# burchim/EfficientConformer

Hardware: AMD Instinct MI355X
Metric: audio-frames/sec through encoder, EffConformerCTC-Small, 1/2/4/8 GPU (higher is better)
Workload: dtype bf16; 1 GPU; EfficientConformerCTCSmall: bf16 operands / fp32 accumulate, B=256 utterances/GPU (the largest single-GPU batch measured; SURVEY.md 8d lists B in {4, 32, 128}: --batch 128 is 0.79 x this rate, profiles/r5_31_bench_b128.json), lognormal 1.5-16 s (LibriSpeech-shaped), sorted desc; ragged: every utterance at its own length in one concatenated row space per row range (no pad frames; outputs = the refe; global_batch=256, streams_per_gpu=3, parallelism=dp1 (utterance shards), row_ranges=3 ragged row range(s) per GPU, cut for equal valid frames

## Files before the change

### efficientconformer_amd/csrc/mel.hip

```cpp
#include "kernels.h"

#ifdef MEL_PK_BUILD
#define launch_mel launch_mel_pk_unused
#define launch_mel_debug launch_mel_debug_pk
#define MEL_NS mel_pk_build
#else
#define MEL_NS
#endif

namespace MEL_NS {

constexpr int NFFT = 512;
constexpr int FRAMES_PER_BLOCK = 32;
constexpr int MAX_MELS = 128;
constexpr int P1 = 72;
constexpr int P2 = 68;
constexpr int MAX_FBW = 768;

__device__ __forceinline__ float2 cmul(float2 a, float2 b) { return make_float2(a.x * b.x - a.y * b.y, a.x * b.y + a.y * b.x); }
__device__ __forceinline__ float2 cadd(float2 a, float2 b) { return make_float2(a.x + b.x, a.y + b.y); }
__device__ __forceinline__ float2 csub(float2 a, float2 b) { return make_float2(a.x - b.x, a.y - b.y); }
__device__ __forceinline__ float2 mul_mi(float2 a) { return make_float2(a.y, -a.x); }
__device__ __forceinline__ float2 mul_pi(float2 a) { return make_float2(-a.y, a.x); }

__device__ __forceinline__ void dft8(float2 (&v)[8]) {
    const float r = 0.70710678118654752f;
    float2 a[4], b[4];
#pragma unroll
    for (int j = 0; j < 4; ++j) { a[j] = cadd(v[j], v[j + 4]); b[j] = csub(v[j], v[j + 4]); }
    b[1] = make_float2(r * (b[1].x + b[1].y), r * (b[1].y - b[1].x));
    b[2] = mul_mi(b[2]);
    b[3] = make_float2(r * (b[3].y - b[3].x), -r * (b[3].x + b[3].y));
    {
        const float2 s0 = cadd(a[0], a[2]), s1 = cadd(a[1], a[3]), d0 = csub(a[0], a[2]), d1 = csub(a[1], a[3]);
        v[0] = cadd(s0, s1); v[4] = csub(s0, s1); v[2] = cadd(d0, mul_mi(d1)); v[6] = cadd(d0, mul_pi(d1));
    }
    {
        const float2 s0 = cadd(b[0], b[2]), s1 = cadd(b[1], b[3]), d0 = csub(b[0], b[2]), d1 = csub(b[1], b[3]);
        v[1] = cadd(s0, s1); v[5] = csub(s0, s1); v[3] = cadd(d0, mul_mi(d1)); v[7] = cadd(d0, mul_pi(d1));
    }
}

__device__ __forceinline__ float2 reread(const float2* p) {
    const volatile float* q = reinterpret_cast<const volatile float*>(p);
    return make_float2(q[0], q[1]);
}

template <int V, int MM>
__global__ __launch_bounds__(256) void mel_kernel(const float* __restrict__ audio, int L, MelTables tb, int hop,
                                                  int n_mels, int Tm, int normalize, float mean, float inv_std,
                                                  float* __restrict__ mel, unsigned int* __restrict__ dbg,
                                                  const int64_t* __restrict__ rag_len = nullptr) {
    constexpr int CAN = (V & 1) ? 512 : 0;
    constexpr int WBUF = 8 * P1 * 8;
    constexpr int O_SBUF = CAN * 4, O_POST = O_SBUF + 4 * WBUF, O_STW = O_POST + CAN * 4, O_SWIN = O_STW + (NFFT / 2) * 8,
                  O_SOUT = O_SWIN + NFFT * 4, O_SFW = O_SOUT + MM * (FRAMES_PER_BLOCK + 1) * 4, O_END = O_SFW + MAX_FBW * 4;
    static_assert(8 * P1 >= NFFT && P1 >= P2 && 8 * P1 * 2 >= 264 + NFFT / 2 + 1, "one buffer holds Z[512], the step-2 layout and the two power spectra");
    __shared__ __attribute__((aligned(16))) char lds[O_END];
    float2* stw = reinterpret_cast<float2*>(lds + O_STW);
    float* swin = reinterpret_cast<float*>(lds + O_SWIN);
    float (*sout)[FRAMES_PER_BLOCK + 1] = reinterpret_cast<float (*)[FRAMES_PER_BLOCK + 1]>(lds + O_SOUT);
    float* sfw = reinterpret_cast<float*>(lds + O_SFW);
    if constexpr ((V & 1) != 0) {
        unsigned int* c0 = reinterpret_cast<unsigned int*>(lds), *c1 = reinterpret_cast<unsigned int*>(lds + O_POST);
        for (int i = threadIdx.x; i < CAN; i += 256) { c0[i] = 0xC0FFEE00u + i; c1[i] = 0xBADC0DE0u + i; }
    }
    auto hand_off = [&]() __attribute__((always_inline)) { if constexpr ((V & 4) != 0) __syncthreads(); else wave_sync(); };
    unsigned int bad[8] = {0, 0, 0, 0, 0, 0, 0, 0};
    auto neq = [](float2 a, float2 b) { return (__float_as_uint(a.x) != __float_as_uint(b.x)) | (__float_as_uint(a.y) != __float_as_uint(b.y)); };
    const int tiles = (Tm + FRAMES_PER_BLOCK - 1) / FRAMES_PER_BLOCK;
    const int b = blockIdx.x / tiles, t0 = (blockIdx.x % tiles) * FRAMES_PER_BLOCK;
    const int Lb = rag_len ? (int)rag_len[b] : L;
    const int Tmb = rag_len ? Lb / hop + 1 : Tm;
    if (t0 >= Tmb) return;
    const int tid = threadIdx.x, lane = tid & 63, wave = tid >> 6;
    const bool fw_lds = tb.fb_nnz <= MAX_FBW;
    {
        static_assert(NFFT == 512 && MAX_FBW == 768, "two / three passes of 256 threads");
        const float2 w = tb.twiddle[tid];
        const float wn0 = tb.window[tid], wn1 = tb.window[tid + 256];
        float f[3];
#pragma unroll
        for (int j = 0; j < 3; ++j) { const int i = tid + 256 * j; f[j] = tb.fb_weight[i < tb.fb_nnz ? i : (tb.fb_nnz > 0 ? tb.fb_nnz - 1 : 0)]; }
        stw[tid] = w;
        swin[tid] = wn0; swin[tid + 256] = wn1;
        if (fw_lds) {
#pragma unroll
            for (int j = 0; j < 3; ++j) if (tid + 256 * j < tb.fb_nnz) sfw[tid + 256 * j] = f[j];
        }
    }
    int fs0[2], fcnt[2], foff[2];
#pragma unroll
    for (int j = 0; j < 2; ++j) {
        const int m = (threadIdx.x & 63) + 64 * j, mc = m < n_mels ? m : n_mels - 1;
        fs0[j] = tb.fb_start[mc]; fcnt[j] = m < n_mels ? tb.fb_count[mc] : 0; foff[j] = tb.fb_offset[mc];
    }
    __syncthreads();
    float2* A = reinterpret_cast<float2*>(lds + O_SBUF + wave * WBUF);
    float2* B = A;
    auto tw = [&](int m) __attribute__((always_inline)) {
        float2 w = stw[m & 255];
        const uint32_t sg = (uint32_t)(m & 256) << 23;
        w.x = __uint_as_float(__float_as_uint(w.x) ^ sg); w.y = __uint_as_float(__float_as_uint(w.y) ^ sg);
        return w;
    };
    const float* a = audio + (size_t)b * L;

    auto gather = [&](int ta, float (&xa)[8], float (&xb)[8]) __attribute__((always_inline)) {
#pragma unroll
        for (int j = 0; j < 8; ++j) {
            const int n = lane + 64 * j;
            int sa = ta * hop - NFFT / 2 + n, sb = sa + hop;
            sa = sa < 0 ? -sa : sa; sa = sa >= Lb ? 2 * (Lb - 1) - sa : sa; sa = sa < 0 ? 0 : (sa >= Lb ? Lb - 1 : sa);
            sb = sb < 0 ? -sb : sb; sb = sb >= Lb ? 2 * (Lb - 1) - sb : sb; sb = sb < 0 ? 0 : (sb >= Lb ? Lb - 1 : sb);
            xa[j] = a[sa]; xb[j] = a[sb];
        }
    };
    float nxa[8], nxb[8];
    gather(t0 + wave * (FRAMES_PER_BLOCK / 4), nxa, nxb);
    for (int it = 0; it < FRAMES_PER_BLOCK / 8; ++it) {
        const int fl = wave * (FRAMES_PER_BLOCK / 4) + 2 * it;
        const int ta = t0 + fl, tbb = ta + 1;
        float2 v[8];
#pragma unroll
        for (int j = 0; j < 8; ++j) {
            const float w = swin[lane + 64 * j];
            v[j] = make_float2(ta < Tmb ? nxa[j] * w : 0.f, tbb < Tmb ? nxb[j] * w : 0.f);
        }
        bool nza = false, nzb = false;
#pragma unroll
        for (int j = 0; j < 8; ++j) { nza |= v[j].x != 0.f; nzb |= v[j].y != 0.f; }
        const bool live_a = __builtin_amdgcn_ballot_w64(nza) != 0, live_b = __builtin_amdgcn_ballot_w64(nzb) != 0;
        if (it + 1 < FRAMES_PER_BLOCK / 8) gather(ta + 2, nxa, nxb);
        {
            const int n2 = lane >> 3;
            dft8(v);
#pragma unroll
            for (int k1 = 0; k1 < 8; ++k1) { v[k1] = cmul(v[k1], tw((8 * n2 * k1) & 511)); A[k1 * P1 + lane] = v[k1]; }
        }
        hand_off();
        if constexpr ((V & 2) != 0) {
#pragma unroll
            for (int k1 = 0; k1 < 8; ++k1) bad[1] += neq(A[k1 * P1 + lane], v[k1]);
        }
        {
            const int k1 = lane >> 3, n3 = lane & 7;
#pragma unroll
            for (int n2 = 0; n2 < 8; ++n2) v[n2] = A[k1 * P1 + n2 * 8 + n3];
            if constexpr ((V & 2) != 0) {
                __builtin_amdgcn_fence(__ATOMIC_ACQUIRE, "wavefront");
#pragma unroll
                for (int n2 = 0; n2 < 8; ++n2) bad[2] += neq(reread(&A[k1 * P1 + n2 * 8 + n3]), v[n2]);
            }
            dft8(v);
#pragma unroll
            for (int k2 = 0; k2 < 8; ++k2) { v[k2] = cmul(v[k2], tw((n3 * (k1 + 8 * k2)) & 511)); B[n3 * P2 + k1 + 8 * k2] = v[k2]; }
        }
        hand_off();
        if constexpr ((V & 2) != 0) {
            const int k1 = lane >> 3, n3 = lane & 7;
#pragma unroll
            for (int k2 = 0; k2 < 8; ++k2) bad[3] += neq(B[n3 * P2 + k1 + 8 * k2], v[k2]);
        }
#pragma unroll
        for (int n3 = 0; n3 < 8; ++n3) v[n3] = B[n3 * P2 + lane];
        if constexpr ((V & 2) != 0) {
            __builtin_amdgcn_fence(__ATOMIC_ACQUIRE, "wavefront");
#pragma unroll
            for (int n3 = 0; n3 < 8; ++n3) bad[4] += neq(reread(&B[n3 * P2 + lane]), v[n3]);
        }
        dft8(v);
#pragma unroll
        for (int k3 = 0; k3 < 8; ++k3) A[lane + 64 * k3] = v[k3];
        hand_off();
        if constexpr ((V & 2) != 0) {
#pragma unroll
            for (int k3 = 0; k3 < 8; ++k3) bad[5] += neq(A[lane + 64 * k3], v[k3]);
        }
        float* Pa = reinterpret_cast<float*>(B);
        float* Pb = Pa + 264;
        float2 zz[5], zcc[5];
#pragma unroll
        for (int j = 0; j < 5; ++j) {
            const int k = lane + 64 * j, kc = k <= NFFT / 2 ? k : NFFT / 2;
            zz[j] = A[kc]; zcc[j] = A[(NFFT - kc) & (NFFT - 1)];
            if constexpr ((V & 2) != 0) {
                __builtin_amdgcn_fence(__ATOMIC_ACQUIRE, "wavefront");
                bad[6] += neq(reread(&A[kc]), zz[j]) + neq(reread(&A[(NFFT - kc) & (NFFT - 1)]), zcc[j]);
            }
        }
        hand_off();
#pragma unroll
        for (int j = 0; j < 5; ++j) {
            const int k = lane + 64 * j;
            if (k <= NFFT / 2) {
                const float2 z = zz[j], zc = zcc[j];
                const float ar = 0.5f * (z.x + zc.x), ai = 0.5f * (z.y - zc.y);
                const float br = 0.5f * (z.y + zc.y), bi = 0.5f * (zc.x - z.x);
                Pa[k] = live_a ? ar * ar + ai * ai : 0.f;
                Pb[k] = live_b ? br * br + bi * bi : 0.f;
            }
        }
        hand_off();
#pragma unroll
        for (int mj = 0; mj < 2; ++mj) {
            const int m = lane + 64 * mj;
            if (m >= n_mels) break;
            const int s0 = fs0[mj], cnt = fcnt[mj], off = foff[mj];
            float ya = 0.f, yb = 0.f;
            if (fw_lds) {
                for (int j0 = 0; j0 < cnt; j0 += 4) {
                    float wj[4], pa[4], pb[4];
#pragma unroll
                    for (int e = 0; e < 4; ++e) {
                        const int j = j0 + e, jc = j < cnt ? j : cnt - 1;
                        wj[e] = j < cnt ? sfw[off + jc] : 0.f;
                        pa[e] = Pa[s0 + jc]; pb[e] = Pb[s0 + jc];
                    }
#pragma unroll
                    for (int e = 0; e < 4; ++e) { ya = fmaf(pa[e], wj[e], ya); yb = fmaf(pb[e], wj[e], yb); }
                }
            } else {
                const float* w = tb.fb_weight + off;
                for (int j = 0; j < cnt; ++j) { const float wj = w[j]; ya = fmaf(Pa[s0 + j], wj, ya); yb = fmaf(Pb[s0 + j], wj, yb); }
            }
            ya = logf(ya + 1e-9f); yb = logf(yb + 1e-9f);
            if (normalize) { ya = (ya - mean) * inv_std; yb = (yb - mean) * inv_std; }
            sout[m][fl] = ya;
            sout[m][fl + 1] = yb;
        }
        hand_off();
    }
    __syncthreads();
    for (int i = tid; i < n_mels * FRAMES_PER_BLOCK; i += 256) {
        const int m = i / FRAMES_PER_BLOCK, fl = i - m * FRAMES_PER_BLOCK;
        if (t0 + fl < Tmb) mel[((size_t)b * n_mels + m) * Tm + t0 + fl] = sout[m][fl];
    }
    if constexpr ((V & 1) != 0) {
        const unsigned int* c0 = reinterpret_cast<const unsigned int*>(lds), *c1 = reinterpret_cast<const unsigned int*>(lds + O_POST);
        for (int i = threadIdx.x; i < CAN; i += 256) bad[0] += (c0[i] != 0xC0FFEE00u + i) + (c1[i] != 0xBADC0DE0u + i);
    }
    if constexpr (V != 0) {
#pragma unroll
        for (int i = 0; i < 8; ++i) if (bad[i]) atomicAdd(dbg + i, bad[i]);
    }
}

}
#ifdef MEL_PK_BUILD
using namespace mel_pk_build;
#endif

int launch_mel(const float* audio, int B, int L, const MelTables& t, int n_fft, int hop, int n_mels, int Tm,
               int normalize, float mean, float std, float* mel, hipStream_t s, const int64_t* ragged_len) {
    if (B <= 0) return 0;
    if (n_fft != NFFT || n_mels > MAX_MELS || L <= n_fft / 2) return -2;
    const int tiles = (Tm + FRAMES_PER_BLOCK - 1) / FRAMES_PER_BLOCK;
    if (n_mels <= 80)
        hipLaunchKernelGGL((mel_kernel<0, 80>), dim3(B * tiles), dim3(256), 0, s, audio, L, t, hop, n_mels, Tm, normalize, mean,
                           1.0f / std, mel, (unsigned int*)nullptr, ragged_len);
    else
        hipLaunchKernelGGL((mel_kernel<0, MAX_MELS>), dim3(B * tiles), dim3(256), 0, s, audio, L, t, hop, n_mels, Tm, normalize, mean,
                           1.0f / std, mel, (unsigned int*)nullptr, ragged_len);
    return hipGetLastError() == hipSuccess ? 0 : -1;
}

#if defined(EFFCONF_DEBUG_ABI) || defined(MEL_PK_BUILD)
int launch_mel_debug(int variant, int extra_lds, const float* audio, int B, int L, const MelTables& t, int n_fft, int hop, int n_mels,
                     int Tm, int normalize, float mean, float std, float* mel, unsigned int* dbg, hipStream_t s) {
    if (B <= 0) return 0;
    if (n_fft != NFFT || n_mels > MAX_MELS || L <= n_fft / 2) return -2;
#ifndef MEL_PK_BUILD
    if (variant & 8) return launch_mel_debug_pk(variant & 7, extra_lds, audio, B, L, t, n_fft, hop, n_mels, Tm, normalize, mean, std, mel, dbg, s);
#endif
    const int tiles = (Tm + FRAMES_PER_BLOCK - 1) / FRAMES_PER_BLOCK;
#define MEL_DBG_CASE(VV) case VV: { static LdsAttr attr; ensure_dynamic_lds(reinterpret_cast<const void*>(&mel_kernel<VV, MAX_MELS>), extra_lds, attr); \
        hipLaunchKernelGGL((mel_kernel<VV, MAX_MELS>), dim3(B * tiles), dim3(256), extra_lds, s, audio, L, t, hop, n_mels, Tm, normalize, mean, 1.0f / std, mel, dbg, (const int64_t*)nullptr); break; }
    switch (variant) {
        MEL_DBG_CASE(0) MEL_DBG_CASE(1) MEL_DBG_CASE(2) MEL_DBG_CASE(3) MEL_DBG_CASE(4) MEL_DBG_CASE(5) MEL_DBG_CASE(6) MEL_DBG_CASE(7)
        default: return -2;
    }
#undef MEL_DBG_CASE
    return hipGetLastError() == hipSuccess ? 0 : -1;
}
#endif
```

Before: 61.85 million mel-frames/s (valid, 10 ms hop).

## Streamline mel kernel: fast-path audio gather, overlap table loads, simplify filterbank loop

Adds a fast path for interior frames that loads audio contiguously without reflect-padding index math, and falls back to the clamped path only at the edges. The first frame gather is issued before the table stores to LDS and the barrier, so global latency overlaps setup. The validity masking moves into the gather, the liveness test becomes an integer OR of bit patterns, and the filterbank loop drops its index clamping by zero-padding the power-spectrum gaps and the weight tail. The mel-to-lane mapping is rebalanced so the tail lanes share work, and the wave index is made wave-uniform. The change adds branch divergence risk between the fast and edge paths and relies on the zeroed gaps for correctness.

```diff
diff --git a/efficientconformer_amd/csrc/mel.hip b/efficientconformer_amd/csrc/mel.hip
--- a/efficientconformer_amd/csrc/mel.hip
+++ b/efficientconformer_amd/csrc/mel.hip
@@ -16,6 +16,7 @@
 constexpr int P1 = 72;
 constexpr int P2 = 68;
 constexpr int MAX_FBW = 768;
+constexpr int FBW_PAD = 4;
 
 __device__ __forceinline__ float2 cmul(float2 a, float2 b) { return make_float2(a.x * b.x - a.y * b.y, a.x * b.y + a.y * b.x); }
 __device__ __forceinline__ float2 cadd(float2 a, float2 b) { return make_float2(a.x + b.x, a.y + b.y); }
@@ -54,8 +55,8 @@
     constexpr int CAN = (V & 1) ? 512 : 0;
     constexpr int WBUF = 8 * P1 * 8;
     constexpr int O_SBUF = CAN * 4, O_POST = O_SBUF + 4 * WBUF, O_STW = O_POST + CAN * 4, O_SWIN = O_STW + (NFFT / 2) * 8,
-                  O_SOUT = O_SWIN + NFFT * 4, O_SFW = O_SOUT + MM * (FRAMES_PER_BLOCK + 1) * 4, O_END = O_SFW + MAX_FBW * 4;
-    static_assert(8 * P1 >= NFFT && P1 >= P2 && 8 * P1 * 2 >= 264 + NFFT / 2 + 1, "one buffer holds Z[512], the step-2 layout and the two power spectra");
+                  O_SOUT = O_SWIN + NFFT * 4, O_SFW = O_SOUT + MM * (FRAMES_PER_BLOCK + 1) * 4, O_END = O_SFW + (MAX_FBW + FBW_PAD) * 4;
+    static_assert(8 * P1 >= NFFT && P1 >= P2 && 8 * P1 * 2 >= 2 * 264, "one buffer holds Z[512], the step-2 layout and the two power spectra with their zeroed gaps");
     __shared__ __attribute__((aligned(16))) char lds[O_END];
     float2* stw = reinterpret_cast<float2*>(lds + O_STW);
     float* swin = reinterpret_cast<float*>(lds + O_SWIN);
@@ -73,27 +74,54 @@
     const int Lb = rag_len ? (int)rag_len[b] : L;
     const int Tmb = rag_len ? Lb / hop + 1 : Tm;
     if (t0 >= Tmb) return;
-    const int tid = threadIdx.x, lane = tid & 63, wave = tid >> 6;
+    const int tid = threadIdx.x, lane = tid & 63;
+    const int wave = __builtin_amdgcn_readfirstlane(tid >> 6);
     const bool fw_lds = tb.fb_nnz <= MAX_FBW;
-    {
-        static_assert(NFFT == 512 && MAX_FBW == 768, "two / three passes of 256 threads");
-        const float2 w = tb.twiddle[tid];
-        const float wn0 = tb.window[tid], wn1 = tb.window[tid + 256];
-        float f[3];
-#pragma unroll
-        for (int j = 0; j < 3; ++j) { const int i = tid + 256 * j; f[j] = tb.fb_weight[i < tb.fb_nnz ? i : (tb.fb_nnz > 0 ? tb.fb_nnz - 1 : 0)]; }
-        stw[tid] = w;
-        swin[tid] = wn0; swin[tid + 256] = wn1;
-        if (fw_lds) {
-#pragma unroll
-            for (int j = 0; j < 3; ++j) if (tid + 256 * j < tb.fb_nnz) sfw[tid + 256 * j] = f[j];
-        }
-    }
-    int fs0[2], fcnt[2], foff[2];
+    static_assert(NFFT == 512 && MAX_FBW == 768, "two / three passes of 256 threads");
+    const float2 w = tb.twiddle[tid];
+    const float wn0 = tb.window[tid], wn1 = tb.window[tid + 256];
+    float f[3];
+#pragma unroll
+    for (int j = 0; j < 3; ++j) { const int i = tid + 256 * j; f[j] = tb.fb_weight[i < tb.fb_nnz ? i : (tb.fb_nnz > 0 ? tb.fb_nnz - 1 : 0)]; }
+    const int mlo = n_mels > 64 ? n_mels - 64 : 0;
+    int fm[2], fs0[2], fcnt[2], foff[2];
 #pragma unroll
     for (int j = 0; j < 2; ++j) {
-        const int m = (threadIdx.x & 63) + 64 * j, mc = m < n_mels ? m : n_mels - 1;
-        fs0[j] = tb.fb_start[mc]; fcnt[j] = m < n_mels ? tb.fb_count[mc] : 0; foff[j] = tb.fb_offset[mc];
+        const int m = j == 0 ? mlo + lane : lane;
+        const bool on = j == 0 ? m < n_mels : lane < mlo;
+        const int mc = on ? m : 0;
+        const int c = tb.fb_count[mc];
+        fm[j] = on ? m : -1; fs0[j] = tb.fb_start[mc]; fcnt[j] = on ? c : 0; foff[j] = tb.fb_offset[mc];
+    }
+    const float* a = audio + (size_t)b * L;
+
+    auto gather = [&](int ta, float (&xa)[8], float (&xb)[8]) __attribute__((always_inline)) {
+        const int base = ta * hop - NFFT / 2;
+        if (base >= 0 && base + hop + NFFT <= Lb) {
+            const float* pa = a + base + lane;
+            const float* pb = pa + hop;
+#pragma unroll
+            for (int j = 0; j < 8; ++j) { xa[j] = pa[64 * j]; xb[j] = pb[64 * j]; }
+        } else {
+            const bool va = ta < Tmb, vb = ta + 1 < Tmb;
+#pragma unroll
+            for (int j = 0; j < 8; ++j) {
+                int sa = base + lane + 64 * j, sb = sa + hop;
+                sa = sa < 0 ? -sa : sa; sa = sa >= Lb ? 2 * (Lb - 1) - sa : sa; sa = sa < 0 ? 0 : (sa >= Lb ? Lb - 1 : sa);
+                sb = sb < 0 ? -sb : sb; sb = sb >= Lb ? 2 * (Lb - 1) - sb : sb; sb = sb < 0 ? 0 : (sb >= Lb ? Lb - 1 : sb);
+                const float ya = a[sa], yb = a[sb];
+                xa[j] = va ? ya : 0.f; xb[j] = vb ? yb : 0.f;
+            }
+        }
+    };
+    float nxa[8], nxb[8];
+    gather(t0 + wave * (FRAMES_PER_BLOCK / 4), nxa, nxb);
+    stw[tid] = w;
+    swin[tid] = wn0; swin[tid + 256] = wn1;
+    if (fw_lds) {
+#pragma unroll
+        for (int j = 0; j < 3; ++j) sfw[tid + 256 * j] = f[j];
+        if (tid < FBW_PAD) sfw[MAX_FBW + tid] = 0.f;
     }
     __syncthreads();
     float2* A = reinterpret_cast<float2*>(lds + O_SBUF + wave * WBUF);
@@ -104,33 +132,19 @@
         w.x = __uint_as_float(__float_as_uint(w.x) ^ sg); w.y = __uint_as_float(__float_as_uint(w.y) ^ sg);
         return w;
     };
-    const float* a = audio + (size_t)b * L;
-
-    auto gather = [&](int ta, float (&xa)[8], float (&xb)[8]) __attribute__((always_inline)) {
-#pragma unroll
-        for (int j = 0; j < 8; ++j) {
-            const int n = lane + 64 * j;
-            int sa = ta * hop - NFFT / 2 + n, sb = sa + hop;
-            sa = sa < 0 ? -sa : sa; sa = sa >= Lb ? 2 * (Lb - 1) - sa : sa; sa = sa < 0 ? 0 : (sa >= Lb ? Lb - 1 : sa);
-            sb = sb < 0 ? -sb : sb; sb = sb >= Lb ? 2 * (Lb - 1) - sb : sb; sb = sb < 0 ? 0 : (sb >= Lb ? Lb - 1 : sb);
-            xa[j] = a[sa]; xb[j] = a[sb];
-        }
-    };
-    float nxa[8], nxb[8];
-    gather(t0 + wave * (FRAMES_PER_BLOCK / 4), nxa, nxb);
     for (int it = 0; it < FRAMES_PER_BLOCK / 8; ++it) {
         const int fl = wave * (FRAMES_PER_BLOCK / 4) + 2 * it;
-        const int ta = t0 + fl, tbb = ta + 1;
+        const int ta = t0 + fl;
         float2 v[8];
 #pragma unroll
         for (int j = 0; j < 8; ++j) {
             const float w = swin[lane + 64 * j];
-            v[j] = make_float2(ta < Tmb ? nxa[j] * w : 0.f, tbb < Tmb ? nxb[j] * w : 0.f);
-        }
-        bool nza = false, nzb = false;
-#pragma unroll
-        for (int j = 0; j < 8; ++j) { nza |= v[j].x != 0.f; nzb |= v[j].y != 0.f; }
-        const bool live_a = __builtin_amdgcn_ballot_w64(nza) != 0, live_b = __builtin_amdgcn_ballot_w64(nzb) != 0;
+            v[j] = make_float2(nxa[j] * w, nxb[j] * w);
+        }
+        uint32_t ua = 0, ub = 0;
+#pragma unroll
+        for (int j = 0; j < 8; ++j) { ua |= __float_as_uint(v[j].x); ub |= __float_as_uint(v[j].y); }
+        const bool live_a = __builtin_amdgcn_ballot_w64((ua & 0x7fffffffu) != 0) != 0, live_b = __builtin_amdgcn_ballot_w64((ub & 0x7fffffffu) != 0) != 0;
         if (it + 1 < FRAMES_PER_BLOCK / 8) gather(ta + 2, nxa, nxb);
         {
             const int n2 = lane >> 3;
@@ -193,29 +207,32 @@
 #pragma unroll
         for (int j = 0; j < 5; ++j) {
             const int k = lane + 64 * j;
-            if (k <= NFFT / 2) {
+            if (j < 4 || lane < 8) {
+                const bool bin = j < 4 || lane == 0;
                 const float2 z = zz[j], zc = zcc[j];
                 const float ar = 0.5f * (z.x + zc.x), ai = 0.5f * (z.y - zc.y);
                 const float br = 0.5f * (z.y + zc.y), bi = 0.5f * (zc.x - z.x);
-                Pa[k] = live_a ? ar * ar + ai * ai : 0.f;
-                Pb[k] = live_b ? br * br + bi * bi : 0.f;
+                Pa[k] = live_a && bin ? ar * ar + ai * ai : 0.f;
+                Pb[k] = live_b && bin ? br * br + bi * bi : 0.f;
             }
         }
         hand_off();
 #pragma unroll
         for (int mj = 0; mj < 2; ++mj) {
-            const int m = lane + 64 * mj;
-            if (m >= n_mels) break;
+            const int m = fm[mj];
+            if (m < 0) continue;
             const int s0 = fs0[mj], cnt = fcnt[mj], off = foff[mj];
             float ya = 0.f, yb = 0.f;
             if (fw_lds) {
+                const float* pp = Pa + s0;
+                const float* pw = sfw + off;
                 for (int j0 = 0; j0 < cnt; j0 += 4) {
                     float wj[4], pa[4], pb[4];
 #pragma unroll
                     for (int e = 0; e < 4; ++e) {
-                        const int j = j0 + e, jc = j < cnt ? j : cnt - 1;
-                        wj[e] = j < cnt ? sfw[off + jc] : 0.f;
-                        pa[e] = Pa[s0 + jc]; pb[e] = Pb[s0 + jc];
+                        const int j = j0 + e;
+                        wj[e] = j < cnt ? pw[j] : 0.f;
+                        pa[e] = pp[j]; pb[e] = pp[264 + j];
                     }
 #pragma unroll
                     for (int e = 0; e < 4; ++e) { ya = fmaf(pa[e], wj[e], ya); yb = fmaf(pb[e], wj[e], yb); }
```

Result: no change. 62.28 million mel-frames/s (valid, 10 ms hop), median of 6 (+0.7%).
